# swarth100/dynfu

Measured on AMD Instinct MI355X. Metric: frames/sec (warp-solve + TSDF fuse), 512^3 vol / 2k nodes / VGA depth, higher is better.
Workload: dtype f32; 1 GPU; C2: 512^3 TSDF, 640x480 depth, 2048 nodes, k=4, 262144 vertices, 5 GN x PCG<=256 (tol 1e-6), reference-parity energy (energy.t), lambda=200; parallelism=replicas x1 (one sequence per GPU, no collective), ranks_seen=1, repeats=5

## Files before the change

### dynfu_amd/csrc/capi.cpp

```cpp
#include <hip/hip_runtime.h>

#include <cmath>
#include <cstdarg>
#include <cstdio>
#include <cstring>
#include <map>
#include <mutex>
#include <new>
#include <utility>
#include <vector>

#include "../../include/dynfu_amd.h"
#include "kernels.hpp"
#include "dev_switch.hpp"
#include "solve.hpp"
#include "solve6.hpp"

namespace {

thread_local char g_err[512] = "";

int fail(int code, const char* fmt, ...) {
    va_list ap;
    va_start(ap, fmt);
    vsnprintf(g_err, sizeof(g_err), fmt, ap);
    va_end(ap);
    return code;
}

int hip_fail(hipError_t e, const char* what) {
    return fail(e == hipErrorNoDevice ? DFA_ERR_NO_GPU : DFA_ERR_HIP, "%s: %s", what, hipGetErrorString(e));
}

#define REQUIRE(cond, msg) \
    if (!(cond)) return fail(DFA_ERR_INVALID, "%s: %s", __func__, msg)
#define HIP_TRY(expr)                                  \
    do {                                               \
// ... 855 lines not shown
        if (rc == DFA_OK && hipHostMalloc((void**)&s->team.host_abort, sizeof(int), hipHostMallocDefault) == hipSuccess) {
            *s->team.host_abort = 0;
            s->team.ctl = s->v.team_ctl;
            if (const char* e0 = dfa::dev_env("DFA_MB_TEAM_EPOCH")) s->team.epoch = (unsigned)std::strtoul(e0, nullptr, 0);
        }
    }
    if (rc == DFA_OK) rc = plan_alloc(s, &s->state, 1);
    if (rc == DFA_OK) rc = plan_alloc(s, &s->iters_total, 1);
    if (rc == DFA_OK && hipMemset(s->iters_total, 0, sizeof(long long)) != hipSuccess) rc = DFA_ERR_HIP;
    if (rc == DFA_OK && hipHostMalloc((void**)&s->host_flag, 4 * sizeof(int), hipHostMallocDefault) != hipSuccess) s->host_flag = nullptr;
    if (rc == DFA_OK) rc = plan_alloc(s, &s->cost_partials, std::max<size_t>((R + 255) / 256 + 1, 1024) + 1024);
    if (rc == DFA_OK) rc = plan_alloc(s, &s->ticket, 64);
    if (rc == DFA_OK && hipMemset(s->ticket, 0, 64 * sizeof(unsigned int)) != hipSuccess)
        rc = fail(DFA_ERR_HIP, "hipMemset (ticket)");
    if (rc != DFA_OK) {
        dfa_solver_destroy(s);
        return rc;
    }
    *out = s;
    return DFA_OK;
}

void dfa_solver_destroy(dfa_solver* s) {
    if (!s) return;
    for (void* p : s->blocks) (void)hipFree(p);
    s->grid.release();
    for (hipEvent_t e : s->events) (void)hipEventDestroy(e);
    if (s->host_flag) (void)hipHostFree(s->host_flag);
    if (s->team.host_abort) (void)hipHostFree(s->team.host_abort);
    s->mb_graphs.release();
    delete s;
}

int dfa_solver_set_problem(dfa_solver* s, const float* node_pos, const float* node_dq, const float* node_w, int D,
                           const float* canon_vertices, const float* canon_normals, const float* live_vertices,
                           const float* live_normals, int N, dfa_stream_t stream) {
    (void)canon_normals;
    (void)live_normals;
    REQUIRE(s, "null plan");
    REQUIRE(node_pos && node_dq && node_w && D > 0, "no nodes");
    REQUIRE(N >= 0 && (N == 0 || (canon_vertices && live_vertices)), "bad vertex arrays");
    if (D > s->max_D || N > s->max_N)
        return fail(DFA_ERR_CAPACITY, "dfa_solver_set_problem: D=%d N=%d exceed the plan (max_D=%d max_N=%d)", D, N,
                    s->max_D, s->max_N);
    dfa::SolveView& v = s->v;
    v.N = N, v.D = D, v.k = s->k, v.Dpad = (D + 3) & ~3, v.ell_cap = s->ell_cap;
    v.deterministic = s->deterministic ? 1 : 0;
    v.node_pos = node_pos, v.node_dq = node_dq, v.node_w = node_w;
    v.canon = canon_vertices, v.live = live_vertices;
    hipStream_t st = S(stream);
    const dfa::KnnGridView* grid = nullptr;
    if (want_grid(D, (long)N + D)) {
        HIP_TRY(dfa::knn_grid_build(s->grid.v, node_pos, D, st));
        grid = &s->grid.v;
    }
    if (N > 0) HIP_TRY(dfa::launch_knn(node_pos, node_w, D, canon_vertices, N, s->k, v.ridx, v.rw, grid, st));
    HIP_TRY(dfa::launch_knn(node_pos, node_w, D, node_pos, D, s->k, v.reg_idx, nullptr, grid, st));
    HIP_TRY(dfa::solve_build_graph(v, s->state, s->ticket, 64, st));
    s->has_problem = true;
    s->just_reset  = true;
    return DFA_OK;
}

int dfa_solver_set_deterministic(dfa_solver* s, int on) {
    REQUIRE(s, "null plan");
    s->deterministic = on != 0;
    return DFA_OK;
}

int dfa_solver_solve(dfa_solver* s, const dfa_solve_params* p, dfa_stream_t stream) {
    REQUIRE(s && p, "null plan / params");
    REQUIRE(s->has_problem, "set_problem has not been called");
    REQUIRE(p->num_iter >= 0 && p->nonlinear_iter >= 0 && p->linear_iter >= 0, "negative iteration count");
    REQUIRE(p->tukey_offset > 0.f && p->psi_data > 0.f, "tukey_offset / psi_data must be positive");
    REQUIRE(p->lambda >= 0.f && std::isfinite(p->lambda), "lambda must be non-negative and finite");
    const dfa::SolveView& v = s->v;
    hipStream_t st          = S(stream);
    if (!s->just_reset) HIP_TRY(dfa::solve_reset(v, s->state, s->ticket, 64, st));
    s->just_reset = false;
    const double w_reg    = std::sqrt((double)p->lambda / ((double)v.D * (double)v.k));
    const float w_reg_f   = (float)w_reg;
    const float w_reg_sq  = w_reg_f * w_reg_f;
    if (s->timing) s->timed_solves += 1;
    if (s->host_flag) s->host_flag[0] = s->host_flag[1] = 0;
    s->mb_graphs.call = 0;
    int not_launched = 0;
    int gn_launched = 0;
    bool huber_done = false;
    const bool big_budget = (long)p->num_iter * p->nonlinear_iter > 8;
    const bool pcg_async  = dfa::solve_pcg_is_async(v, &s->team, p->linear_iter);
    const bool no_regradient = dfa::dev_env("DFA_NO_REGRADIENT") != nullptr;
// ... 503 lines not shown
```

### dynfu_amd/csrc/solve.hip

```cpp
#include <hip/hip_runtime.h>
#include <cstring>

#include <algorithm>
#include <map>
#include <mutex>

#include <float.h>

#include "dq_device.hpp"
#include "dev_switch.hpp"
#include "kernels.hpp"
#include "pcg_rules.hpp"
#include "solve.hpp"

namespace dfa {


constexpr int TG_BLOCKS = SOLVE_TG_BLOCKS;

__global__ __launch_bounds__(1024) void tg_count_kernel(const int32_t* __restrict__ ridx, size_t total, int D,
                                                        int32_t* __restrict__ blk_hist ) {
    extern __shared__ int32_t hist[];
    for (int i = threadIdx.x; i < D; i += blockDim.x) hist[i] = 0;
    __syncthreads();
// ... 250 lines not shown
    }
    if (threadIdx.x == 0) {
        const double cost = sm[0];
        if (a.update_weights) st->amax = (float)smx[0];
        if (!st->have_initial) st->initial_cost = cost, st->have_initial = 1;
        if (a.mode == 0) st->done = 0;
        if (a.mode == 1 && !st->done && a.gn_tol > 0.f && (st->cost - cost) <= (double)a.gn_tol * st->cost)
            st->done = 1;
        st->cost       = cost;
        st->final_cost = cost;
        st->cost_stale = 0;
        if (a.mode != 2) st->weights_fresh = a.update_weights;
        if (a.mode != 2 && a.update_weights && st->converged == 2) st->converged = 0;
    }
}

__global__ __launch_bounds__(256) void reset_kernel(float* __restrict__ t, int n3, SolveState* __restrict__ st,
                                                    unsigned int* __restrict__ ticket, int nticket) {
    const int i = blockIdx.x * blockDim.x + threadIdx.x;
    if (i < n3) t[i] = 0.f;
    if (blockIdx.x == 0) {
        unsigned int* w = (unsigned int*)st;
        for (int j = threadIdx.x; j < (int)(sizeof(SolveState) / 4); j += blockDim.x) w[j] = 0u;
        for (int j = threadIdx.x; j < nticket; j += blockDim.x) ticket[j] = 0u;
    }
}

template <int K>
__global__ __launch_bounds__(256) void prepare_rows_kernel(SolveView s, SolveState* __restrict__ st,
                                                           unsigned int* __restrict__ ticket, int nticket) {
    const size_t R = (size_t)s.N + (size_t)s.D * s.k;
    const size_t r = (size_t)blockIdx.x * blockDim.x + threadIdx.x;
    if (r < (size_t)3 * s.D) s.t[r] = 0.f;
    if (blockIdx.x == 0) {
        unsigned int* w = (unsigned int*)st;
        for (int j = threadIdx.x; j < (int)(sizeof(SolveState) / 4); j += blockDim.x) w[j] = 0u;
        for (int j = threadIdx.x; j < nticket; j += blockDim.x) ticket[j] = 0u;
    }
    if (r >= R) return;
    const int k = s.k;
    int ids[K];
    float ws[K];
    const bool wide = k == K && K % 4 == 0;
    if (r < (size_t)s.N) {
#pragma unroll
        for (int c = 0; c < 3; ++c) s.rb[3 * r + c] = s.live[3 * r + c] - s.canon[3 * r + c];
        if (wide) load_row_graph<K>(s, r, ids, ws);
        else {
#pragma unroll
            for (int j = 0; j < K; ++j)
                if (j < k) ids[j] = s.ridx[r * k + j], ws[j] = s.rw[r * k + j];
        }
    } else {
        const int e = (int)(r - (size_t)s.N), n = e / k, m = s.reg_idx[e];
#pragma unroll
        for (int j = 0; j < K; ++j) ids[j] = -1, ws[j] = 0.f;
        if (m >= 0 && m != n) ids[0] = m, ws[0] = -1.f, ids[1] = n, ws[1] = +1.f;
        if (wide) {
#pragma unroll
            for (int q = 0; q < K / 4; ++q) {
                reinterpret_cast<int4*>(s.ridx + r * K)[q]  = make_int4(ids[4 * q], ids[4 * q + 1], ids[4 * q + 2], ids[4 * q + 3]);
                reinterpret_cast<float4*>(s.rw + r * K)[q] = make_float4(ws[4 * q], ws[4 * q + 1], ws[4 * q + 2], ws[4 * q + 3]);
            }
        } else {
#pragma unroll
            for (int j = 0; j < K; ++j)
                if (j < k) s.ridx[r * k + j] = ids[j], s.rw[r * k + j] = ws[j];
        }
        s.rb[3 * r + 0] = s.rb[3 * r + 1] = s.rb[3 * r + 2] = 0.f;
    }
    float* rec = s.re + r * (size_t)solve_rec_words(k);
    if (wide) {
        float4* rec4 = reinterpret_cast<float4*>(rec);
        if (solve_rec_ids16(k)) {
            uint32_t pk[K / 2];
#pragma unroll
            for (int j = 0; j < K / 2; ++j) {
                const uint32_t lo = ids[2 * j] < 0 ? 0xffffu : (uint32_t)ids[2 * j], hi = ids[2 * j + 1] < 0 ? 0xffffu : (uint32_t)ids[2 * j + 1];
                pk[j]             = (lo & 0xffffu) | (hi << 16);
            }
#pragma unroll
            for (int q = 0; q < K / 8; ++q)
                rec4[q] = make_float4(__uint_as_float(pk[4 * q]), __uint_as_float(pk[4 * q + 1]), __uint_as_float(pk[4 * q + 2]), __uint_as_float(pk[4 * q + 3]));
#pragma unroll
            for (int q = 0; q < K / 4; ++q) rec4[K / 8 + q] = make_float4(ws[4 * q], ws[4 * q + 1], ws[4 * q + 2], ws[4 * q + 3]);
        } else {
#pragma unroll
            for (int q = 0; q < K / 4; ++q)
                rec4[q] = make_float4(__int_as_float(ids[4 * q]), __int_as_float(ids[4 * q + 1]), __int_as_float(ids[4 * q + 2]), __int_as_float(ids[4 * q + 3]));
#pragma unroll
            for (int q = 0; q < K / 4; ++q) rec4[K / 4 + q] = make_float4(ws[4 * q], ws[4 * q + 1], ws[4 * q + 2], ws[4 * q + 3]);
        }
        return;
    }
    if (solve_rec_ids16(k)) {
        uint16_t* h = reinterpret_cast<uint16_t*>(rec);
#pragma unroll
        for (int j = 0; j < K; ++j)
            if (j < k) h[j] = ids[j] < 0 ? (uint16_t)0xffffu : (uint16_t)ids[j], rec[k / 2 + j] = ws[j];
        return;
    }
#pragma unroll
    for (int j = 0; j < K; ++j)
        if (j < k) rec[j] = __int_as_float(ids[j]), rec[k + j] = ws[j];
}


constexpr int HASH      = 512;
constexpr int HASH_MASK = HASH - 1;

struct FixedScale {
    float up;
    double down;
};
__device__ __forceinline__ FixedScale solve_fixed_scale(float amax) {
    int e = 0;
    (void)frexpf(fmaxf(amax, 1e-30f), &e);
    e = e < -80 ? -80 : e > 100 ? 100 : e;
    FixedScale f;
    f.up   = ldexpf(1.f, 40 - e);
    f.down = ldexp(1.0, e - 40);
    return f;
}
__device__ __forceinline__ FixedScale fixed_scale_for_rows(FixedScale f, int rows) {
    const int extra = 32 - __clz((unsigned)max(rows, 1) >> 22);
    if (extra > 0) f.up = ldexpf(f.up, -extra), f.down = ldexp(f.down, extra);
    return f;
}
__device__ __forceinline__ void fixed_add(long long* cell, float v, float up) {
    const float x  = truncf(fabsf(v) * up);
    const float hf = floorf(x * 2.3283064365386963e-10f);
    const uint32_t hi = (uint32_t)hf, lo = (uint32_t)fmaf(hf, -4294967296.f, x);
    atomicAdd(reinterpret_cast<unsigned long long*>(v < 0.f ? cell + HASH : cell), ((unsigned long long)hi << 32) | lo);
}

template <int K>
__device__ __forceinline__ float4 load_record(const SolveView& s, size_t r, int (&idx)[K], float (&w)[K]) {
// ... 924 lines not shown
#endif
#pragma unroll
    for (int j = 0; j < P; ++j)
#pragma unroll
        for (int c = 0; c < NC; ++c) {
            if (rowA[j] >= 0) s.t[3 * rowA[j] + c0 + c] += xA[j][c];
            if (rowB[j] >= 0) s.t[3 * rowB[j] + c0 + c] += xB[j][c];
        }
    if (tid == 0) {
        if (NC == 3) pcg_book_launch(st, rz0, it, false);
        else pcg_book_launch_of_three(st, rz0, it, false);
    }
}


#define KDISPATCH(kernel, k, ...)                      \
    do {                                               \
        if ((k) <= 4) kernel<4> __VA_ARGS__;           \
        else if ((k) <= 8) kernel<8> __VA_ARGS__;      \
        else kernel<16> __VA_ARGS__;                   \
    } while (0)

hipError_t solve_transpose_graph(const int32_t* ridx, size_t total, int D, int32_t* blk_hist, int32_t* node_ptr,
                                 uint32_t* node_list, hipStream_t st) {
    const size_t lds = sizeof(int32_t) * (size_t)D;
    tg_count_kernel<<<TG_BLOCKS, 1024, lds, st>>>(ridx, total, D, blk_hist);
    tg_colscan_kernel<<<(D + 255) / 256, 256, 0, st>>>(blk_hist, D);
    tg_fill_kernel<<<TG_BLOCKS, 1024, lds, st>>>(ridx, total, D, blk_hist, node_ptr, node_list);
    return hipGetLastError();
}

hipError_t solve_build_graph(const SolveView& s, SolveState* state, unsigned int* ticket, int nticket, hipStream_t st) {
    const int D = s.D, N = s.N, k = s.k;
    const size_t R = (size_t)N + (size_t)D * k, total = R * k;
    const size_t threads = R > (size_t)3 * D ? R : (size_t)3 * D;
    KDISPATCH(prepare_rows_kernel, k, <<<(unsigned)((threads + 255) / 256), 256, 0, st>>>(s, state, ticket, nticket));
    const size_t lds = sizeof(int32_t) * (size_t)D;
    tg_count_kernel<<<TG_BLOCKS, 1024, lds, st>>>(s.ridx, total, D, s.blk_hist);
    tg_colscan_kernel<<<(D + 255) / 256, 256, 0, st>>>(s.blk_hist, D);
    tg_fill_kernel<<<TG_BLOCKS, 1024, lds, st>>>(s.ridx, total, D, s.blk_hist, s.node_ptr, s.node_list);
    if (s.deterministic) sort_node_lists_kernel<<<D, 256, 0, st>>>(s.node_ptr, s.node_list);
    return hipGetLastError();
}

int solve_residual_blocks(const SolveView& s) {
    const size_t R  = (size_t)s.N + (size_t)s.D * s.k;
    const size_t nb = (R + 255) / 256;
    return (int)(nb < (size_t)LIN_MAX_BLOCKS ? nb : (size_t)LIN_MAX_BLOCKS);
}

hipError_t solve_linearise(const SolveView& s, SolveState* state, double* cost_partials, unsigned int* ticket,
                           int update_weights, int mode, float gn_tol, float tukey_offset, float psi_data,
                           float w_reg_sq, float huber_psi, long long* iters_total, hipStream_t st) {
    const int nb = solve_residual_blocks(s);
    LineariseArgs a{update_weights, mode, gn_tol, tukey_offset, psi_data, w_reg_sq, iters_total, huber_psi};
    KDISPATCH(linearise_kernel, s.k, <<<nb, 256, 0, st>>>(s, state, cost_partials, ticket, a));
    return hipGetLastError();
}

hipError_t solve_reset(const SolveView& s, SolveState* state, unsigned int* ticket, int nticket, hipStream_t st) {
    reset_kernel<<<(3 * s.D + 255) / 256, 256, 0, st>>>(s.t, 3 * s.D, state, ticket, nticket);
    return hipGetLastError();
}

hipError_t solve_huber(const SolveView& s, float psi_reg, hipStream_t st) {
    huber_kernel<<<(s.D + 255) / 256, 256, 0, st>>>(s, psi_reg);
    return hipGetLastError();
}

// ... 783 lines not shown
```

### dynfu_amd/csrc/solve.hpp

```cpp
#pragma once
#include <hip/hip_runtime.h>
#include <stdint.h>

namespace dfa {

struct SolveState {
    double initial_cost;
    double cost;
    double final_cost;
    double grad_first;
    int have_initial;
    int done;
    int gn_iters;
    int pcg_iters;
    int max_row_nnz;
    int overflow;
    int pcg_fallback;
    int split_iters;
    unsigned int split_ticket;
    int mb_done;
    int converged;
    int mb_skip, mb_iters;
    int weights_fresh;
    int gn_noop;
// ... 29 lines not shown
    const float* node_w;
    const float* canon;
    const float* live;
    int32_t* ridx;
    float* rw;
    float* rtau;
    float* rb;
    float* re;
    int32_t* reg_idx;
    int32_t* blk_hist;
    int32_t* node_ptr;
    uint32_t* node_list;
    float2* ell;
    int32_t* ell_cnt;
    float* diag;
    float* g;
    float* g_base;
    float* t_base;
    int32_t* pk_perm;
    int32_t* pk_perm2;
    float* pk_vals;
    uint16_t* pk_cols;
    float4 *mb_x, *mb_r, *mb_p, *mb_s, *mb_w, *mb_u[2], *mb_m[2], *mb_t[2];
    float *mb_gpart[2], *mb_dpart[2];
    TeamCtl* team_ctl;
    float2* team_mt;
    unsigned long long* team_words;
    int team_stride;
    float* t;
    float* huber;
    float* node_dq_out;
};

constexpr int SOLVE_TG_BLOCKS = 256;
hipError_t solve_build_graph(const SolveView& s, SolveState* state, unsigned int* ticket, int nticket, hipStream_t st);
hipError_t solve_transpose_graph(const int32_t* ridx, size_t total, int D, int32_t* blk_hist, int32_t* node_ptr,
                                 uint32_t* node_list, hipStream_t st);
int solve_residual_blocks(const SolveView& s);
hipError_t solve_linearise(const SolveView& s, SolveState* state, double* cost_partials, unsigned int* ticket,
                           int update_weights, int mode, float gn_tol, float tukey_offset, float psi_data,
                           float w_reg_sq, float huber_psi ,
                           long long* iters_total , hipStream_t st);
hipError_t solve_huber(const SolveView& s, float psi_reg, hipStream_t st);
hipError_t solve_reset(const SolveView& s, SolveState* state, unsigned int* ticket, int nticket, hipStream_t st);
hipError_t solve_assemble(const SolveView& s, SolveState* state, int save_base , float w_reg_sq,
                          hipStream_t st);
hipError_t solve_regradient(const SolveView& s, SolveState* state, hipStream_t st);
int solve_pcg_max_nodes();
__host__ __device__ inline int solve_mb_rows_per_block() { return 16; }
__host__ __device__ inline int solve_mb_blocks(int D) { return (D + 15) / 16; }
struct MbGraphCache {
    struct Entry {
        int it0 = 0, it1 = 0;
        float tol = 0.f;
        SolveView view;
        const SolveState* state = nullptr;
        hipGraphExec_t exec = nullptr;
    };
    Entry e[24];
    int used = 0;
    int pred[64] = {};
    int call     = 0;
    hipStream_t capture = nullptr;
    bool disabled = false;
    void release();
};

struct TeamPcg {
// ... 18 lines not shown
```

### dynfu_amd/csrc/warp.hip

```cpp
#include <hip/hip_runtime.h>

#include "dq_device.hpp"
#include "dev_switch.hpp"
#include "kernels.hpp"

namespace dfa {

constexpr int KNN_TILE = 1024;

template <int K>
struct KnnList {
    unsigned long long key[K];
    static constexpr unsigned long long EMPTY = 0x7f8000007fffffffull;
    __device__ __forceinline__ static unsigned long long pack(float dist, int idx) {
        return ((unsigned long long)__float_as_uint(dist) << 32) | (unsigned int)idx;
    }
    __device__ __forceinline__ void init() {
#pragma unroll
        for (int j = 0; j < K; ++j) key[j] = EMPTY;
    }
    __device__ __forceinline__ void push(float dist, int idx) {
        const unsigned long long x = pack(dist, idx);
        if (x < key[K - 1]) {
            key[K - 1] = x;
#pragma unroll
            for (int j = K - 1; j > 0; --j) {
                const unsigned long long a = key[j - 1], b = key[j];
                key[j - 1] = a < b ? a : b, key[j] = a < b ? b : a;
            }
        }
    }
    __device__ __forceinline__ float dist(int j) const { return __uint_as_float((unsigned int)(key[j] >> 32)); }
    __device__ __forceinline__ int raw_index(int j) const { return (int)(unsigned int)key[j]; }
    __device__ __forceinline__ int index(int j) const { return raw_index(j) == 0x7fffffff ? -1 : raw_index(j); }
    __device__ __forceinline__ void set_index(int j, int n) { key[j] = pack(__builtin_inff(), n < 0 ? 0x7fffffff : n); }
};

// ... 504 lines not shown
    for (int r = r_first; r < rmax; ++r) {
        const int z0 = max(cz - r, 0), z1 = min(cz + r, g.dim[2] - 1);
        const int y0 = max(cy - r, 0), y1 = min(cy + r, g.dim[1] - 1);
        const int x0 = max(cx - r, 0), x1 = min(cx + r, g.dim[0] - 1);
        for (int z = z0; z <= z1; ++z)
            for (int y = y0; y <= y1; ++y) {
                const bool face = (abs(z - cz) == r) || (abs(y - cy) == r);
                const int xstep = face ? 1 : max(x1 - x0, 1);
                for (int x = x0; x <= x1; x += xstep) {
                    if (!face && abs(x - cx) != r) continue;
                    const int c   = x + g.dim[0] * (y + g.dim[1] * z);
                    const int beg = cell_start[c], end = cell_start[c + 1];
                    for (int j = beg; j < end; ++j) {
                        const float4 n = sorted[j];
                        best.push(dist2(q, n.x, n.y, n.z), __float_as_int(n.w));
                    }
                }
            }
        const float bound = TIGHT ? fmaxf((float)r + margin - 1e-3f, 0.f) * g.cs : (float)r * g.cs;
        if (best.dist(K - 1) < bound * bound * 0.9999f) break;
    }
}

__device__ __forceinline__ unsigned long long wave_min_u64(unsigned long long v) {
#pragma unroll
    for (int o = 32; o > 0; o >>= 1) {
        const unsigned long long t = __shfl_xor(v, o, 64);
        v                          = t < v ? t : v;
    }
    return v;
}

template <int K>
__global__ __launch_bounds__(256) void knn_wave_kernel(const float* __restrict__ node_pos,
                                                       const float* __restrict__ node_w, int D,
                                                       const float* __restrict__ query, int n_query, int k,
                                                       int32_t* __restrict__ idx, float* __restrict__ weights,
                                                       KnnGridView grid) {
    const int v    = blockIdx.x * 4 + (threadIdx.x >> 6);
    const int lane = threadIdx.x & 63;
    if (v >= n_query) return;
    const KnnGridDesc g = *grid.desc;
    const f3 q = mk3(query[3 * (size_t)v], query[3 * (size_t)v + 1], query[3 * (size_t)v + 2]);
    KnnList<K> best;
    best.init();
    int cx, cy, cz;
    cell_of(g, q, cx, cy, cz);
    const int rmax = max(g.dim[0], max(g.dim[1], g.dim[2]));
    for (int r = 0; r < rmax; ++r) {
        const int side = 2 * r + 1, ncell = side * side * side;
        for (int c = lane; c < ncell; c += 64) {
            const int dx = c % side - r, dy = (c / side) % side - r, dz = c / (side * side) - r;
            if (max(abs(dx), max(abs(dy), abs(dz))) != r) continue;
            const int x = cx + dx, y = cy + dy, z = cz + dz;
            if (x < 0 || y < 0 || z < 0 || x >= g.dim[0] || y >= g.dim[1] || z >= g.dim[2]) continue;
            const int cell = x + g.dim[0] * (y + g.dim[1] * z);
            const int beg = grid.cell_start[cell], end = grid.cell_start[cell + 1];
            for (int j = beg; j < end; ++j) {
                const float4 n = grid.sorted[j];
                best.push(dist2(q, n.x, n.y, n.z), __float_as_int(n.w));
            }
        }
        const float bound = (float)r * g.cs, b2 = bound * bound * 0.9999f;
        int inside = 0;
#pragma unroll
        for (int j = 0; j < K; ++j) inside += best.dist(j) < b2 ? 1 : 0;
#pragma unroll
        for (int o = 32; o > 0; o >>= 1) inside += __shfl_xor(inside, o, 64);
        if (inside >= K) break;
    }
    int pos = 0;
    for (int j = 0; j < K; ++j) {
        unsigned long long key = KnnList<K>::EMPTY;
#pragma unroll
        for (int t = 0; t < K; ++t)
            if (t == pos) key = best.key[t];
        const int hi = (int)(unsigned int)key;
        const unsigned long long win = wave_min_u64(key);
        if (key == win && hi != 0x7fffffff) ++pos;
        if (lane == 0 && j < k) {
            const int n            = (int)(win & 0xffffffffu);
            const int node         = n == 0x7fffffff ? -1 : n;
            idx[(size_t)v * k + j] = node;
            if (weights) {
                float w = 0.f;
                if (node >= 0)
                    w = transformation_weight(mk3(node_pos[3 * node], node_pos[3 * node + 1], node_pos[3 * node + 2]),
                                              node_w[node], q);
                weights[(size_t)v * k + j] = w;
            }
        }
    }
}

template <int K, bool GRID>
__global__ __launch_bounds__(256) void knn_kernel(const float* __restrict__ node_pos,
                                                  const float* __restrict__ node_w, int D,
                                                  const float* __restrict__ query, int n_query, int k,
                                                  int32_t* __restrict__ idx, float* __restrict__ weights,
                                                  KnnGridView grid) {
    __shared__ float4 tile[GRID ? 1 : KNN_TILE];
    const int v       = blockIdx.x * blockDim.x + threadIdx.x;
    const bool active = v < n_query;
    f3 q              = mk3(0.f, 0.f, 0.f);
    if (active) q = mk3(query[3 * (size_t)v], query[3 * (size_t)v + 1], query[3 * (size_t)v + 2]);
    KnnList<K> best;
    if (GRID) {
        if (!active) return;
        knn_grid_query<K>(*grid.desc, grid.cell_start, grid.sorted, q, best);
    } else {
        knn_scan<K>(node_pos, D, q, best, tile);
        if (!active) return;
    }
    int out_i[K];
    float out_w[K];
#pragma unroll
    for (int j = 0; j < K; ++j) {
        out_i[j] = -1, out_w[j] = 0.f;
        if (j < k) {
            const int n = best.index(j);
            out_i[j]    = n;
            if (weights && n >= 0)
                out_w[j] = transformation_weight(mk3(node_pos[3 * n], node_pos[3 * n + 1], node_pos[3 * n + 2]), node_w[n], q);
        }
    }
    if (k == K && K % 4 == 0 && ((reinterpret_cast<uintptr_t>(idx) | reinterpret_cast<uintptr_t>(weights)) & 15u) == 0) {
#pragma unroll
        for (int h = 0; h < K / 4; ++h) {
            reinterpret_cast<int4*>(idx + (size_t)v * K)[h] = make_int4(out_i[4 * h], out_i[4 * h + 1], out_i[4 * h + 2], out_i[4 * h + 3]);
            if (weights)
                reinterpret_cast<float4*>(weights + (size_t)v * K)[h] = make_float4(out_w[4 * h], out_w[4 * h + 1], out_w[4 * h + 2], out_w[4 * h + 3]);
        }
        return;
    }
#pragma unroll
    for (int j = 0; j < K; ++j)
        if (j < k) {
            idx[(size_t)v * k + j] = out_i[j];
            if (weights) weights[(size_t)v * k + j] = out_w[j];
        }
}

template <int K>
__device__ __forceinline__ DQ calc_dqb(const KnnList<K>& nb, int k, const float* __restrict__ node_pos,
                                       const float* __restrict__ node_dq, const float* __restrict__ node_w, f3 p) {
    DQ sum = dq_identity();
    constexpr int G = K < 4 ? K : 4;
#pragma unroll
    for (int h = 0; h < K; h += G) {
        f3 g[G];
        float r[G];
        DQ q[G];
        bool on[G];
#pragma unroll
        for (int jj = 0; jj < G; ++jj) {
            const int j = h + jj;
            on[jj]      = j < k && nb.index(j) >= 0;
            const int n = on[jj] ? nb.index(j) : 0;
            g[jj] = mk3(node_pos[3 * n], node_pos[3 * n + 1], node_pos[3 * n + 2]), r[jj] = node_w[n];
            q[jj] = dq_load(node_dq + 8 * (size_t)n);
        }
#pragma unroll
        for (int jj = 0; jj < G; ++jj)
            if (on[jj]) sum = dq_mul(sum, dq_scale(q[jj], transformation_weight(g[jj], r[jj], p)));
    }
    return dq_normalize(sum);
}

template <int K, bool GRID>
__global__ __launch_bounds__(256) void warp_to_live_kernel(const float* __restrict__ node_pos,
                                                           const float* __restrict__ node_dq,
                                                           const float* __restrict__ node_w, int D, int k,
                                                           const float* __restrict__ verts,
// ... 149 lines not shown
    pgrid_scan_kernel<<<chunks, 256, 0, s>>>(g.desc, g.cell_count, g.cell_start, pg.chunk_sums);
    grid_fill_kernel<<<nb, 256, 0, s>>>(pts, n, g.node_cell, g.cell_count, g.sorted);
    return hipGetLastError();
}

hipError_t knn_grid_build(const KnnGridView& g, const float* node_pos, int D, hipStream_t s) {
    if (D <= GRID_ONE_MAX) {
        constexpr size_t lds = sizeof(int32_t) * KNN_GRID_MAX_CELLS;
        hipError_t e = allow_dynamic_lds((const void*)grid_build_one_kernel, (int)lds);
        if (e != hipSuccess) return e;
        grid_build_one_kernel<<<1, 1024, lds, s>>>(node_pos, D, g.desc, g.cell_start, g.sorted);
        return hipGetLastError();
    }
    grid_setup_kernel<<<1, 1024, 0, s>>>(node_pos, D, g.desc, g.cell_count);
    grid_count_kernel<<<(D + 255) / 256, 256, 0, s>>>(node_pos, D, g.desc, g.cell_count, g.node_cell);
    grid_scan_kernel<<<1, 1024, 0, s>>>(g.cell_count, g.cell_start);
    grid_fill_kernel<<<(D + 255) / 256, 256, 0, s>>>(node_pos, D, g.node_cell, g.cell_count, g.sorted);
    return hipGetLastError();
}

#define KGDISPATCH(kernel, k, use_grid, ...)                         \
    do {                                                             \
        if (use_grid) {                                              \
            if ((k) <= 4) kernel<4, true> __VA_ARGS__;               \
            else if ((k) <= 8) kernel<8, true> __VA_ARGS__;          \
            else kernel<16, true> __VA_ARGS__;                       \
        } else {                                                     \
            if ((k) <= 4) kernel<4, false> __VA_ARGS__;              \
            else if ((k) <= 8) kernel<8, false> __VA_ARGS__;         \
            else kernel<16, false> __VA_ARGS__;                      \
        }                                                            \
    } while (0)

hipError_t launch_knn(const float* node_pos, const float* node_w, int D, const float* query, int n_query, int k,
                      int32_t* idx, float* weights, const KnnGridView* grid, hipStream_t s) {
    if (n_query == 0) return hipSuccess;
    dim3 block(256), gridDim((n_query + 255) / 256);
    const bool use_grid = grid != nullptr;
    KnnGridView g       = use_grid ? *grid : KnnGridView{};
    if (use_grid && n_query <= 32768) {
        dim3 wgrid((n_query + 3) / 4);
        if (k <= 4) knn_wave_kernel<4><<<wgrid, block, 0, s>>>(node_pos, node_w, D, query, n_query, k, idx, weights, g);
        else if (k <= 8) knn_wave_kernel<8><<<wgrid, block, 0, s>>>(node_pos, node_w, D, query, n_query, k, idx, weights, g);
        else knn_wave_kernel<16><<<wgrid, block, 0, s>>>(node_pos, node_w, D, query, n_query, k, idx, weights, g);
        return hipGetLastError();
    }
    KGDISPATCH(knn_kernel, k, use_grid, <<<gridDim, block, 0, s>>>(node_pos, node_w, D, query, n_query, k, idx, weights, g));
    return hipGetLastError();
}

hipError_t launch_warp_to_live(const float* node_pos, const float* node_dq, const float* node_w, int D, int k,
                               const float* verts, const float* normals, int N, float* out_verts, float* out_normals,
                               const KnnGridView* grid, hipStream_t s) {
    if (N == 0) return hipSuccess;
    dim3 block(256), gridDim((N + 255) / 256);
    const bool use_grid = grid != nullptr;
    KnnGridView g       = use_grid ? *grid : KnnGridView{};
    KGDISPATCH(warp_to_live_kernel, k, use_grid,
               <<<gridDim, block, 0, s>>>(node_pos, node_dq, node_w, D, k, verts, normals, N, out_verts, out_normals, g));
    return hipGetLastError();
}

__global__ __launch_bounds__(256) void correspond_projective_kernel(const float* __restrict__ verts,
                                                                    const float* __restrict__ normals, int n,
                                                                    const float* __restrict__ vmap, int vmap_step,
                                                                    const float* __restrict__ nmap, int nmap_step, int cols,
                                                                    int rows, float fx, float fy, float cx, float cy,
                                                                    float dist2_thres, float min_cosine,
                                                                    float* __restrict__ out_v, float* __restrict__ out_n,
                                                                    int32_t* __restrict__ out_pixel) {
    const int i = blockIdx.x * blockDim.x + threadIdx.x;
    if (i >= n) return;
    const float qn = __uint_as_float(0x7fc00000u);
    const f3 s     = mk3(verts[3 * (size_t)i], verts[3 * (size_t)i + 1], verts[3 * (size_t)i + 2]);
    f3 d = mk3(qn, qn, qn), nd = mk3(qn, qn, qn);
    int pix = -1;
    if (s.z > 0.f) {
        const float u = fmaf(fx, s.x / s.z, cx), w = fmaf(fy, s.y / s.z, cy);
        if (u >= 0.f && w >= 0.f && u < (float)cols && w < (float)rows) {
            const int iu = (int)floorf(u), iw = (int)floorf(w);
// ... 82 lines not shown
```

Baseline: 1594 frames/s.

## Fuse vertex/node KNN and row preparation into one graph-build kernel

In set_problem, the vertex KNN, the node-to-node KNN and the prepare_rows kernel used to run as three launches. When a grid is present, D is small and N is large, they now run as one heterogeneous kernel. Node blocks use the wave-cooperative grid search and write the regularisation rows directly. Vertex blocks run the per-thread grid KNN and write the data rows, weights, records and residual bases without the intermediate ridx/rw round trip. This removes launch overhead and a pass over the row buffers, at the cost of a more complex kernel that mixes two work types in one launch.

```diff
diff --git a/dynfu_amd/csrc/capi.cpp b/dynfu_amd/csrc/capi.cpp
--- a/dynfu_amd/csrc/capi.cpp
+++ b/dynfu_amd/csrc/capi.cpp
@@ -3,6 +3,7 @@
 #include <cmath>
 #include <cstdarg>
 #include <cstdio>
+#include <atomic>
 #include <cstring>
 #include <map>
 #include <mutex>
@@ -924,6 +925,11 @@
     delete s;
 }
 
+#ifdef DFA_DEV_AB
+static std::atomic<long> g_dev_fused_graph_builds{0};
+__attribute__((visibility("default"))) long dfa_dev_fused_graph_builds() { return g_dev_fused_graph_builds.load(); }
+#endif
+
 int dfa_solver_set_problem(dfa_solver* s, const float* node_pos, const float* node_dq, const float* node_w, int D,
                            const float* canon_vertices, const float* canon_normals, const float* live_vertices,
                            const float* live_normals, int N, dfa_stream_t stream) {
@@ -946,9 +952,19 @@
         HIP_TRY(dfa::knn_grid_build(s->grid.v, node_pos, D, st));
         grid = &s->grid.v;
     }
-    if (N > 0) HIP_TRY(dfa::launch_knn(node_pos, node_w, D, canon_vertices, N, s->k, v.ridx, v.rw, grid, st));
-    HIP_TRY(dfa::launch_knn(node_pos, node_w, D, node_pos, D, s->k, v.reg_idx, nullptr, grid, st));
-    HIP_TRY(dfa::solve_build_graph(v, s->state, s->ticket, 64, st));
+    bool fused = dfa::solve_rows_fusable(D, N, grid != nullptr);
+    if (const char* e = dfa::dev_env("DFA_GRAPH_BUILD")) fused = fused && std::strcmp(e, "chain") != 0;
+    if (fused) {
+        HIP_TRY(dfa::solve_build_rows_fused(v, *grid, s->state, s->ticket, 64, st));
+#ifdef DFA_DEV_AB
+        ++g_dev_fused_graph_builds;
+#endif
+        HIP_TRY(dfa::solve_transpose_rows(v, st));
+    } else {
+        if (N > 0) HIP_TRY(dfa::launch_knn(node_pos, node_w, D, canon_vertices, N, s->k, v.ridx, v.rw, grid, st));
+        HIP_TRY(dfa::launch_knn(node_pos, node_w, D, node_pos, D, s->k, v.reg_idx, nullptr, grid, st));
+        HIP_TRY(dfa::solve_build_graph(v, s->state, s->ticket, 64, st));
+    }
     s->has_problem = true;
     s->just_reset  = true;
     return DFA_OK;
diff --git a/dynfu_amd/csrc/solve.hip b/dynfu_amd/csrc/solve.hip
--- a/dynfu_amd/csrc/solve.hip
+++ b/dynfu_amd/csrc/solve.hip
@@ -306,11 +306,7 @@
     const size_t R = (size_t)s.N + (size_t)s.D * s.k;
     const size_t r = (size_t)blockIdx.x * blockDim.x + threadIdx.x;
     if (r < (size_t)3 * s.D) s.t[r] = 0.f;
-    if (blockIdx.x == 0) {
-        unsigned int* w = (unsigned int*)st;
-        for (int j = threadIdx.x; j < (int)(sizeof(SolveState) / 4); j += blockDim.x) w[j] = 0u;
-        for (int j = threadIdx.x; j < nticket; j += blockDim.x) ticket[j] = 0u;
-    }
+    if (blockIdx.x == 0) solve_zero_state(st, ticket, nticket);
     if (r >= R) return;
     const int k = s.k;
     int ids[K];
@@ -327,56 +323,11 @@
         }
     } else {
         const int e = (int)(r - (size_t)s.N), n = e / k, m = s.reg_idx[e];
-#pragma unroll
-        for (int j = 0; j < K; ++j) ids[j] = -1, ws[j] = 0.f;
-        if (m >= 0 && m != n) ids[0] = m, ws[0] = -1.f, ids[1] = n, ws[1] = +1.f;
-        if (wide) {
-#pragma unroll
-            for (int q = 0; q < K / 4; ++q) {
-                reinterpret_cast<int4*>(s.ridx + r * K)[q]  = make_int4(ids[4 * q], ids[4 * q + 1], ids[4 * q + 2], ids[4 * q + 3]);
-                reinterpret_cast<float4*>(s.rw + r * K)[q] = make_float4(ws[4 * q], ws[4 * q + 1], ws[4 * q + 2], ws[4 * q + 3]);
-            }
-        } else {
-#pragma unroll
-            for (int j = 0; j < K; ++j)
-                if (j < k) s.ridx[r * k + j] = ids[j], s.rw[r * k + j] = ws[j];
-        }
+        solve_reg_row<K>(m, n, ids, ws);
+        solve_store_row_graph<K>(s, r, ids, ws);
         s.rb[3 * r + 0] = s.rb[3 * r + 1] = s.rb[3 * r + 2] = 0.f;
     }
-    float* rec = s.re + r * (size_t)solve_rec_words(k);
-    if (wide) {
-        float4* rec4 = reinterpret_cast<float4*>(rec);
-        if (solve_rec_ids16(k)) {
-            uint32_t pk[K / 2];
-#pragma unroll
-            for (int j = 0; j < K / 2; ++j) {
-                const uint32_t lo = ids[2 * j] < 0 ? 0xffffu : (uint32_t)ids[2 * j], hi = ids[2 * j + 1] < 0 ? 0xffffu : (uint32_t)ids[2 * j + 1];
-                pk[j]             = (lo & 0xffffu) | (hi << 16);
-            }
-#pragma unroll
-            for (int q = 0; q < K / 8; ++q)
-                rec4[q] = make_float4(__uint_as_float(pk[4 * q]), __uint_as_float(pk[4 * q + 1]), __uint_as_float(pk[4 * q + 2]), __uint_as_float(pk[4 * q + 3]));
-#pragma unroll
-            for (int q = 0; q < K / 4; ++q) rec4[K / 8 + q] = make_float4(ws[4 * q], ws[4 * q + 1], ws[4 * q + 2], ws[4 * q + 3]);
-        } else {
-#pragma unroll
-            for (int q = 0; q < K / 4; ++q)
-                rec4[q] = make_float4(__int_as_float(ids[4 * q]), __int_as_float(ids[4 * q + 1]), __int_as_float(ids[4 * q + 2]), __int_as_float(ids[4 * q + 3]));
-#pragma unroll
-            for (int q = 0; q < K / 4; ++q) rec4[K / 4 + q] = make_float4(ws[4 * q], ws[4 * q + 1], ws[4 * q + 2], ws[4 * q + 3]);
-        }
-        return;
-    }
-    if (solve_rec_ids16(k)) {
-        uint16_t* h = reinterpret_cast<uint16_t*>(rec);
-#pragma unroll
-        for (int j = 0; j < K; ++j)
-            if (j < k) h[j] = ids[j] < 0 ? (uint16_t)0xffffu : (uint16_t)ids[j], rec[k / 2 + j] = ws[j];
-        return;
-    }
-#pragma unroll
-    for (int j = 0; j < K; ++j)
-        if (j < k) rec[j] = __int_as_float(ids[j]), rec[k + j] = ws[j];
+    solve_store_row_head<K>(s, r, ids, ws);
 }
 
 
@@ -1367,9 +1318,15 @@
 
 hipError_t solve_build_graph(const SolveView& s, SolveState* state, unsigned int* ticket, int nticket, hipStream_t st) {
     const int D = s.D, N = s.N, k = s.k;
-    const size_t R = (size_t)N + (size_t)D * k, total = R * k;
+    const size_t R = (size_t)N + (size_t)D * k;
     const size_t threads = R > (size_t)3 * D ? R : (size_t)3 * D;
     KDISPATCH(prepare_rows_kernel, k, <<<(unsigned)((threads + 255) / 256), 256, 0, st>>>(s, state, ticket, nticket));
+    return solve_transpose_rows(s, st);
+}
+
+hipError_t solve_transpose_rows(const SolveView& s, hipStream_t st) {
+    const int D = s.D;
+    const size_t total = ((size_t)s.N + (size_t)D * s.k) * s.k;
     const size_t lds = sizeof(int32_t) * (size_t)D;
     tg_count_kernel<<<TG_BLOCKS, 1024, lds, st>>>(s.ridx, total, D, s.blk_hist);
     tg_colscan_kernel<<<(D + 255) / 256, 256, 0, st>>>(s.blk_hist, D);
diff --git a/dynfu_amd/csrc/solve.hpp b/dynfu_amd/csrc/solve.hpp
--- a/dynfu_amd/csrc/solve.hpp
+++ b/dynfu_amd/csrc/solve.hpp
@@ -85,8 +85,83 @@
     float* node_dq_out;
 };
 
+
+template <int K>
+__device__ __forceinline__ void solve_reg_row(int m, int n, int (&ids)[K], float (&ws)[K]) {
+#pragma unroll
+    for (int j = 0; j < K; ++j) ids[j] = -1, ws[j] = 0.f;
+    if (m >= 0 && m != n) ids[0] = m, ws[0] = -1.f, ids[1] = n, ws[1] = +1.f;
+}
+
+__device__ __forceinline__ void solve_zero_state(SolveState* st, unsigned int* ticket, int nticket) {
+    unsigned int* w = (unsigned int*)st;
+    for (int j = threadIdx.x; j < (int)(sizeof(SolveState) / 4); j += blockDim.x) w[j] = 0u;
+    for (int j = threadIdx.x; j < nticket; j += blockDim.x) ticket[j] = 0u;
+}
+
+template <int K>
+__device__ __forceinline__ void solve_store_row_graph(const SolveView& s, size_t r, const int (&ids)[K], const float (&ws)[K]) {
+    const int k = s.k;
+    if (k == K && K % 4 == 0) {
+#pragma unroll
+        for (int q = 0; q < K / 4; ++q) {
+            reinterpret_cast<int4*>(s.ridx + r * K)[q]  = make_int4(ids[4 * q], ids[4 * q + 1], ids[4 * q + 2], ids[4 * q + 3]);
+            reinterpret_cast<float4*>(s.rw + r * K)[q] = make_float4(ws[4 * q], ws[4 * q + 1], ws[4 * q + 2], ws[4 * q + 3]);
+        }
+    } else {
+#pragma unroll
+        for (int j = 0; j < K; ++j)
+            if (j < k) s.ridx[r * k + j] = ids[j], s.rw[r * k + j] = ws[j];
+    }
+}
+
+template <int K>
+__device__ __forceinline__ void solve_store_row_head(const SolveView& s, size_t r, const int (&ids)[K], const float (&ws)[K]) {
+    const int k     = s.k;
+    const bool wide = k == K && K % 4 == 0;
+    float* rec = s.re + r * (size_t)solve_rec_words(k);
+    if (wide) {
+        float4* rec4 = reinterpret_cast<float4*>(rec);
+        if (solve_rec_ids16(k)) {
+            uint32_t pk[K / 2];
+#pragma unroll
+            for (int j = 0; j < K / 2; ++j) {
+                const uint32_t lo = ids[2 * j] < 0 ? 0xffffu : (uint32_t)ids[2 * j], hi = ids[2 * j + 1] < 0 ? 0xffffu : (uint32_t)ids[2 * j + 1];
+                pk[j]             = (lo & 0xffffu) | (hi << 16);
+            }
+#pragma unroll
+            for (int q = 0; q < K / 8; ++q)
+                rec4[q] = make_float4(__uint_as_float(pk[4 * q]), __uint_as_float(pk[4 * q + 1]), __uint_as_float(pk[4 * q + 2]), __uint_as_float(pk[4 * q + 3]));
+#pragma unroll
+            for (int q = 0; q < K / 4; ++q) rec4[K / 8 + q] = make_float4(ws[4 * q], ws[4 * q + 1], ws[4 * q + 2], ws[4 * q + 3]);
+        } else {
+#pragma unroll
+            for (int q = 0; q < K / 4; ++q)
+                rec4[q] = make_float4(__int_as_float(ids[4 * q]), __int_as_float(ids[4 * q + 1]), __int_as_float(ids[4 * q + 2]), __int_as_float(ids[4 * q + 3]));
+#pragma unroll
+            for (int q = 0; q < K / 4; ++q) rec4[K / 4 + q] = make_float4(ws[4 * q], ws[4 * q + 1], ws[4 * q + 2], ws[4 * q + 3]);
+        }
+        return;
+    }
+    if (solve_rec_ids16(k)) {
+        uint16_t* h = reinterpret_cast<uint16_t*>(rec);
+#pragma unroll
+        for (int j = 0; j < K; ++j)
+            if (j < k) h[j] = ids[j] < 0 ? (uint16_t)0xffffu : (uint16_t)ids[j], rec[k / 2 + j] = ws[j];
+        return;
+    }
+#pragma unroll
+    for (int j = 0; j < K; ++j)
+        if (j < k) rec[j] = __int_as_float(ids[j]), rec[k + j] = ws[j];
+}
+
 constexpr int SOLVE_TG_BLOCKS = 256;
 hipError_t solve_build_graph(const SolveView& s, SolveState* state, unsigned int* ticket, int nticket, hipStream_t st);
+hipError_t solve_transpose_rows(const SolveView& s, hipStream_t st);
+struct KnnGridView;
+bool solve_rows_fusable(int D, int N, bool grid);
+hipError_t solve_build_rows_fused(const SolveView& s, const KnnGridView& grid, SolveState* state, unsigned int* ticket,
+                                  int nticket, hipStream_t st);
 hipError_t solve_transpose_graph(const int32_t* ridx, size_t total, int D, int32_t* blk_hist, int32_t* node_ptr,
                                  uint32_t* node_list, hipStream_t st);
 int solve_residual_blocks(const SolveView& s);
diff --git a/dynfu_amd/csrc/warp.hip b/dynfu_amd/csrc/warp.hip
--- a/dynfu_amd/csrc/warp.hip
+++ b/dynfu_amd/csrc/warp.hip
@@ -3,6 +3,7 @@
 #include "dq_device.hpp"
 #include "dev_switch.hpp"
 #include "kernels.hpp"
+#include "solve.hpp"
 
 namespace dfa {
 
@@ -573,17 +574,7 @@
 }
 
 template <int K>
-__global__ __launch_bounds__(256) void knn_wave_kernel(const float* __restrict__ node_pos,
-                                                       const float* __restrict__ node_w, int D,
-                                                       const float* __restrict__ query, int n_query, int k,
-                                                       int32_t* __restrict__ idx, float* __restrict__ weights,
-                                                       KnnGridView grid) {
-    const int v    = blockIdx.x * 4 + (threadIdx.x >> 6);
-    const int lane = threadIdx.x & 63;
-    if (v >= n_query) return;
-    const KnnGridDesc g = *grid.desc;
-    const f3 q = mk3(query[3 * (size_t)v], query[3 * (size_t)v + 1], query[3 * (size_t)v + 2]);
-    KnnList<K> best;
+__device__ __forceinline__ void knn_wave_search(const KnnGridDesc& g, const KnnGridView& grid, f3 q, int lane, KnnList<K>& best) {
     best.init();
     int cx, cy, cz;
     cell_of(g, q, cx, cy, cz);
@@ -610,6 +601,10 @@
         for (int o = 32; o > 0; o >>= 1) inside += __shfl_xor(inside, o, 64);
         if (inside >= K) break;
     }
+}
+
+template <int K, typename Emit>
+__device__ __forceinline__ void knn_wave_merge(const KnnList<K>& best, Emit emit) {
     int pos = 0;
     for (int j = 0; j < K; ++j) {
         unsigned long long key = KnnList<K>::EMPTY;
@@ -619,9 +614,26 @@
         const int hi = (int)(unsigned int)key;
         const unsigned long long win = wave_min_u64(key);
         if (key == win && hi != 0x7fffffff) ++pos;
+        const int n = (int)(win & 0xffffffffu);
+        emit(j, n == 0x7fffffff ? -1 : n);
+    }
+}
+
+template <int K>
+__global__ __launch_bounds__(256) void knn_wave_kernel(const float* __restrict__ node_pos,
+                                                       const float* __restrict__ node_w, int D,
+                                                       const float* __restrict__ query, int n_query, int k,
+                                                       int32_t* __restrict__ idx, float* __restrict__ weights,
+                                                       KnnGridView grid) {
+    const int v    = blockIdx.x * 4 + (threadIdx.x >> 6);
+    const int lane = threadIdx.x & 63;
+    if (v >= n_query) return;
+    const KnnGridDesc g = *grid.desc;
+    const f3 q = mk3(query[3 * (size_t)v], query[3 * (size_t)v + 1], query[3 * (size_t)v + 2]);
+    KnnList<K> best;
+    knn_wave_search<K>(g, grid, q, lane, best);
+    knn_wave_merge<K>(best, [&](int j, int node) {
         if (lane == 0 && j < k) {
-            const int n            = (int)(win & 0xffffffffu);
-            const int node         = n == 0x7fffffff ? -1 : n;
             idx[(size_t)v * k + j] = node;
             if (weights) {
                 float w = 0.f;
@@ -630,6 +642,21 @@
                                               node_w[node], q);
                 weights[(size_t)v * k + j] = w;
             }
+        }
+    });
+}
+
+template <int K>
+__device__ __forceinline__ void knn_list_out(const KnnList<K>& best, int k, bool with_w, const float* __restrict__ node_pos,
+                                             const float* __restrict__ node_w, f3 q, int (&out_i)[K], float (&out_w)[K]) {
+#pragma unroll
+    for (int j = 0; j < K; ++j) {
+        out_i[j] = -1, out_w[j] = 0.f;
+        if (j < k) {
+            const int n = best.index(j);
+            out_i[j]    = n;
+            if (with_w && n >= 0)
+                out_w[j] = transformation_weight(mk3(node_pos[3 * n], node_pos[3 * n + 1], node_pos[3 * n + 2]), node_w[n], q);
         }
     }
 }
@@ -655,16 +682,7 @@
     }
     int out_i[K];
     float out_w[K];
-#pragma unroll
-    for (int j = 0; j < K; ++j) {
-        out_i[j] = -1, out_w[j] = 0.f;
-        if (j < k) {
-            const int n = best.index(j);
-            out_i[j]    = n;
-            if (weights && n >= 0)
-                out_w[j] = transformation_weight(mk3(node_pos[3 * n], node_pos[3 * n + 1], node_pos[3 * n + 2]), node_w[n], q);
-        }
-    }
+    knn_list_out<K>(best, k, weights != nullptr, node_pos, node_w, q, out_i, out_w);
     if (k == K && K % 4 == 0 && ((reinterpret_cast<uintptr_t>(idx) | reinterpret_cast<uintptr_t>(weights)) & 15u) == 0) {
 #pragma unroll
         for (int h = 0; h < K / 4; ++h) {
@@ -680,6 +698,49 @@
             idx[(size_t)v * k + j] = out_i[j];
             if (weights) weights[(size_t)v * k + j] = out_w[j];
         }
+}
+
+template <int K>
+__global__ __launch_bounds__(256) void graph_rows_kernel(SolveView s, KnnGridView grid, SolveState* __restrict__ st,
+                                                         unsigned int* __restrict__ ticket, int nticket, int node_blocks) {
+    const int k = s.k;
+    if ((int)blockIdx.x < node_blocks) {
+        if (blockIdx.x == 0) solve_zero_state(st, ticket, nticket);
+        const int n    = blockIdx.x * 4 + (threadIdx.x >> 6);
+        const int lane = threadIdx.x & 63;
+        if (n >= s.D) return;
+        if (lane < 3) s.t[3 * n + lane] = 0.f;
+        const KnnGridDesc g = *grid.desc;
+        const f3 q = mk3(s.node_pos[3 * (size_t)n], s.node_pos[3 * (size_t)n + 1], s.node_pos[3 * (size_t)n + 2]);
+        KnnList<K> best;
+        knn_wave_search<K>(g, grid, q, lane, best);
+        int m = -1;
+        knn_wave_merge<K>(best, [&](int j, int node) {
+            if (lane == j) m = node;
+        });
+        if (lane >= k) return;
+        const size_t e = (size_t)n * k + lane, r = (size_t)s.N + e;
+        s.reg_idx[e] = m;
+        int ids[K];
+        float ws[K];
+        solve_reg_row<K>(m, n, ids, ws);
+        solve_store_row_graph<K>(s, r, ids, ws);
+        s.rb[3 * r + 0] = s.rb[3 * r + 1] = s.rb[3 * r + 2] = 0.f;
+        solve_store_row_head<K>(s, r, ids, ws);
+        return;
+    }
+    const int vi = (blockIdx.x - node_blocks) * blockDim.x + threadIdx.x;
+    if (vi >= s.N) return;
+    const f3 q = mk3(s.canon[3 * (size_t)vi], s.canon[3 * (size_t)vi + 1], s.canon[3 * (size_t)vi + 2]);
+    KnnList<K> best;
+    knn_grid_query<K>(*grid.desc, grid.cell_start, grid.sorted, q, best);
+    int ids[K];
+    float ws[K];
+    knn_list_out<K>(best, k, true, s.node_pos, s.node_w, q, ids, ws);
+    const size_t v = (size_t)((blockIdx.x - node_blocks) * blockDim.x + threadIdx.x);
+    solve_store_row_graph<K>(s, v, ids, ws);
+    solve_store_row_head<K>(s, v, ids, ws);
+    s.rb[3 * v + 0] = s.live[3 * v + 0] - q.x, s.rb[3 * v + 1] = s.live[3 * v + 1] - q.y, s.rb[3 * v + 2] = s.live[3 * v + 2] - q.z;
 }
 
 template <int K>
@@ -895,13 +956,15 @@
         }                                                            \
     } while (0)
 
+constexpr int KNN_WAVE_MAX_QUERIES = 32768;
+
 hipError_t launch_knn(const float* node_pos, const float* node_w, int D, const float* query, int n_query, int k,
                       int32_t* idx, float* weights, const KnnGridView* grid, hipStream_t s) {
     if (n_query == 0) return hipSuccess;
     dim3 block(256), gridDim((n_query + 255) / 256);
     const bool use_grid = grid != nullptr;
     KnnGridView g       = use_grid ? *grid : KnnGridView{};
-    if (use_grid && n_query <= 32768) {
+    if (use_grid && n_query <= KNN_WAVE_MAX_QUERIES) {
         dim3 wgrid((n_query + 3) / 4);
         if (k <= 4) knn_wave_kernel<4><<<wgrid, block, 0, s>>>(node_pos, node_w, D, query, n_query, k, idx, weights, g);
         else if (k <= 8) knn_wave_kernel<8><<<wgrid, block, 0, s>>>(node_pos, node_w, D, query, n_query, k, idx, weights, g);
@@ -909,6 +972,18 @@
         return hipGetLastError();
     }
     KGDISPATCH(knn_kernel, k, use_grid, <<<gridDim, block, 0, s>>>(node_pos, node_w, D, query, n_query, k, idx, weights, g));
+    return hipGetLastError();
+}
+
+bool solve_rows_fusable(int D, int N, bool grid) { return grid && D <= KNN_WAVE_MAX_QUERIES && N > KNN_WAVE_MAX_QUERIES; }
+
+hipError_t solve_build_rows_fused(const SolveView& s, const KnnGridView& grid, SolveState* state, unsigned int* ticket,
+                                  int nticket, hipStream_t st) {
+    const int node_blocks = (s.D + 3) / 4;
+    const unsigned blocks = (unsigned)node_blocks + (unsigned)((s.N + 255) / 256);
+    if (s.k <= 4) graph_rows_kernel<4><<<blocks, 256, 0, st>>>(s, grid, state, ticket, nticket, node_blocks);
+    else if (s.k <= 8) graph_rows_kernel<8><<<blocks, 256, 0, st>>>(s, grid, state, ticket, nticket, node_blocks);
+    else graph_rows_kernel<16><<<blocks, 256, 0, st>>>(s, grid, state, ticket, nticket, node_blocks);
     return hipGetLastError();
 }
 
```

New measurement: 1631 frames/s (median of 6 runs). 1.02x the previous value.
